# DanielaCourel/smoothed_particle_hydrodynamics

Hardware: AMD Instinct MI355X
Metric: Mparticle-steps/sec (whole node), dam-break (higher is better)
Workload: dtype f32

## Files before the change

smoothed_particle_hydrodynamics_amd/csrc/cell_build.h:

```cpp
#pragma once

#include "sph_device.h"

#define SCAN_THREADS 256
#ifndef RANK_UNROLL
#define RANK_UNROLL 4
#endif
#ifndef RANK_BIG
#define RANK_BIG 512
#endif
#define RANK_CHUNK 4096
#define RANK_BIG_BLOCKS 64
#define SCAN_ITEMS 16
#define SCAN_TILE (SCAN_THREADS * SCAN_ITEMS)

__device__ __forceinline__ void count_cell_runs(uint32_t c, bool live, int i,
                                                uint32_t* __restrict__ cell_count,
                                                uint32_t* __restrict__ slot, uint32_t trash)
{
   live = live && c != trash;
   const int lane = threadIdx.x & (SPH_WAVE - 1);
   const uint32_t prev = __shfl_up(c, 1);
   const bool head = (lane == 0) || (prev != c);
   const unsigned long long heads = __ballot(head);
   const unsigned long long below = heads & ((lane == 63) ? ~0ull : ((1ull << (lane + 1)) - 1ull));
   const int head_lane = 63 - __clzll(below);
   const unsigned long long above = (head_lane == 63) ? 0ull : (heads >> (head_lane + 1));
   const int run_len = above ? (__ffsll((long long)above)) : (SPH_WAVE - head_lane);
   uint32_t base = 0;
   if (live && head) base = atomicAdd(&cell_count[c], (uint32_t)run_len);
   base = __shfl(base, head_lane);
   if (live) slot[i] = base + (uint32_t)(lane - head_lane);
}

template <bool WRITE_VOX, bool CHECK_DEAD>
__global__ void __launch_bounds__(256)
k_hash_count(const float4* __restrict__ posm, const float4* __restrict__ velp,
             int32_t* __restrict__ meta, CellGrid g, SlabZone zone, uint32_t* __restrict__ key,
             uint32_t* __restrict__ slot, uint32_t* __restrict__ cell_count,
             int32_t* __restrict__ vox)
{
   const int i = blockIdx.x * blockDim.x + threadIdx.x;
   const bool live = i < meta[META_N_IN];
   uint32_t c = 0xffffffffu;
   if (live) {
      const float4 p = posm[i];
      int cx, cy, cz;
      c = cell_of(g, p.x, p.y, p.z, cx, cy, cz);
      const bool carried = zone.drop_ghosts && i < meta[META_N_LIVE];
      const int ob = meta[META_OWN_BEGIN], oe = meta[META_OWN_END];
      const bool was_owned = i >= ob && i < oe;
      if (CHECK_DEAD && __float_as_uint(velp[i].w) == SPH_DEAD_ID) {
         c = (uint32_t)g.ncells;
      } else if (carried && !was_owned) {
         c = (uint32_t)g.ncells;
// ... 4 lines not shown
         const int hi_begin = max(meta[META_BND_HI_BEGIN], lo_end);
         if (i >= lo_end && i < hi_begin) {
            const int plane = cell_coord(p.z, g.inv, g.nz_global);
            if ((zone.have_left && plane < zone.lo + zone.halo) ||
                (zone.have_right && plane >= zone.hi - zone.halo))
               atomicOr(&meta[META_ERRORS], 8);
         }
      }
      key[i] = c;
      if (WRITE_VOX) {
         vox[3 * i + 0] = cx;
         vox[3 * i + 1] = cy;
         vox[3 * i + 2] = cz;
      }
   }
   count_cell_runs(c, live, i, cell_count, slot, (uint32_t)g.ncells);
}

__device__ __forceinline__ uint32_t wave_inclusive_scan(uint32_t v, int lane)
{
#pragma unroll
   for (int d = 1; d < SPH_WAVE; d <<= 1) {
      uint32_t t = __shfl_up(v, d);
      if (lane >= d) v += t;
   }
   return v;
}

__device__ __forceinline__ uint32_t block_exclusive_scan(uint32_t v, uint32_t* total)
{
   __shared__ uint32_t wave_sums[SCAN_THREADS / SPH_WAVE];
// ... 3 lines not shown
   if (lane == SPH_WAVE - 1) wave_sums[w] = inc;
   __syncthreads();
   uint32_t carry = 0, tot = 0;
#pragma unroll
   for (int k = 0; k < SCAN_THREADS / SPH_WAVE; k++) {
      const uint32_t s = wave_sums[k];
      if (k < w) carry += s;
      tot += s;
   }
   __syncthreads();
   *total = tot;
   return carry + inc - v;
}

__global__ void __launch_bounds__(SCAN_THREADS)
k_scan_reduce(const uint32_t* __restrict__ count, int ncells, uint32_t* __restrict__ part)
{
   const int base = blockIdx.x * SCAN_TILE + threadIdx.x * SCAN_ITEMS;
   uint32_t s = 0;
   if (base + SCAN_ITEMS <= ncells) {
      const uint4* p = reinterpret_cast<const uint4*>(count + base);
#pragma unroll
      for (int k = 0; k < SCAN_ITEMS / 4; k++) {
         const uint4 v = p[k];
         s += v.x + v.y + v.z + v.w;
      }
   } else {
      for (int k = 0; k < SCAN_ITEMS; k++)
         if (base + k < ncells) s += count[base + k];
   }
   uint32_t total;
   block_exclusive_scan(s, &total);
   if (threadIdx.x == 0) part[blockIdx.x] = total;
}

__global__ void __launch_bounds__(SCAN_THREADS)
k_scan_final(uint32_t* __restrict__ count, int ncells, const uint32_t* __restrict__ part,
             uint32_t* __restrict__ cell_start, uint32_t* __restrict__ big_cells, uint32_t limit,
             int32_t* __restrict__ meta)
{
   if (blockIdx.x == 0 && threadIdx.x == 0) big_cells[0] = 0u;
   const int base = blockIdx.x * SCAN_TILE + threadIdx.x * SCAN_ITEMS;
   uint32_t v[SCAN_ITEMS];
   uint32_t s = 0;
   const bool empty_tile = part[blockIdx.x] == 0u;
   if (empty_tile) {
#pragma unroll
      for (int k = 0; k < SCAN_ITEMS; k++) v[k] = 0u;
   } else if (base + SCAN_ITEMS <= ncells) {
      const uint4* p = reinterpret_cast<const uint4*>(count + base);
#pragma unroll
      for (int k = 0; k < SCAN_ITEMS / 4; k++) {
         const uint4 q = p[k];
         v[4 * k + 0] = q.x;
         v[4 * k + 1] = q.y;
         v[4 * k + 2] = q.z;
         v[4 * k + 3] = q.w;
      }
   } else {
#pragma unroll
      for (int k = 0; k < SCAN_ITEMS; k++) v[k] = (base + k < ncells) ? count[base + k] : 0u;
   }
#pragma unroll
   for (int k = 0; k < SCAN_ITEMS; k++) s += v[k];
   uint32_t before = 0;
   for (int t = threadIdx.x; t < (int)blockIdx.x; t += SCAN_THREADS) before += part[t];
   uint32_t carry;
   block_exclusive_scan(before, &carry);
   uint32_t total;
   uint32_t run = carry + block_exclusive_scan(s, &total);
   if (base + SCAN_ITEMS <= ncells) {
      uint4* o = reinterpret_cast<uint4*>(cell_start + base);
      uint4* z = reinterpret_cast<uint4*>(count + base);
#pragma unroll
      for (int k = 0; k < SCAN_ITEMS / 4; k++) {
         uint4 q;
         q.x = min(run, limit); run += v[4 * k + 0];
         q.y = min(run, limit); run += v[4 * k + 1];
         q.z = min(run, limit); run += v[4 * k + 2];
         q.w = min(run, limit); run += v[4 * k + 3];
         o[k] = q;
         if ((v[4 * k + 0] | v[4 * k + 1] | v[4 * k + 2] | v[4 * k + 3]) != 0u) z[k] = make_uint4(0, 0, 0, 0);
      }
   } else {
      for (int k = 0; k < SCAN_ITEMS; k++) {
         if (base + k < ncells) {
            cell_start[base + k] = min(run, limit);
            if (v[k] != 0u) count[base + k] = 0;
            run += v[k];
         }
      }
   }
   if (base <= ncells - 1 && ncells - 1 < base + SCAN_ITEMS) {
      cell_start[ncells] = min(run, limit);
      if (run > limit) atomicOr(&meta[META_ERRORS], 4);
   }
}

__global__ void __launch_bounds__(256)
k_scatter(const uint32_t* __restrict__ key, const uint32_t* __restrict__ slot,
          const uint32_t* __restrict__ cell_start, int32_t* __restrict__ meta,
          uint32_t* __restrict__ perm, int cells_per_plane, int ncells, int own_lo, int own_hi,
          int sum_lo, int sum_hi, int bnd_lo, int bnd_hi, int32_t* __restrict__ tile_stats,
          int32_t* __restrict__ clear_a, int32_t* __restrict__ clear_b,
          uint32_t* __restrict__ big_cells, uint32_t limit)
{
   const int i = blockIdx.x * blockDim.x + threadIdx.x;
   if (tile_stats && i < TSTAT_COUNT && i != TSTAT_BLOCKS) tile_stats[i] = 0;
// ... 236 lines not shown
```

smoothed_particle_hydrodynamics_amd/csrc/common_kernels.h:

```cpp
#pragma once

#include "body_policy.h"
#include "cell_build.h"
#include "load_policy.h"
#include "obstacle_policy.h"
#include "pair_math.h"

#define RED_THREADS 256

__device__ __forceinline__ void apply_boundary(const PairConsts& k, const float pos[3], float dt,
                                               float np[3], float dist, int axis, float sgn,
                                               float nv[3])
{
   float normal[3] = {0.0f, 0.0f, 0.0f};
   normal[axis] = sgn;
   float inter[3], refl[3];
#pragma unroll
   for (int c = 0; c < 3; c++) inter[c] = pos[c] + (nv[c] * dist);
   const float dot = nv[0] * normal[0] + nv[1] * normal[1] + nv[2] * normal[2];
#pragma unroll
   for (int c = 0; c < 3; c++) refl[c] = nv[c] - ((normal[c] * dot) * 2.0f);
   const float remaining = dt - dist;
#pragma unroll
   for (int c = 0; c < 3; c++) {
// ... 183 lines not shown
   }
};

template <bool UNIT_SCALE>
__device__ __forceinline__ void integrate_particle(const PairConsts& k, float4& x, float4& v,
                                                   const float4 a, double& ke, double& pe)
{
   integrate_particle_hooked<UNIT_SCALE>(k, x, v, a, ke, pe, NoHook());
}

template <bool UNIT_SCALE, bool HASH, class Hook>
__device__ __forceinline__ void integrate_block(float4* __restrict__ posm, float4* __restrict__ velp,
                                                const float4* __restrict__ acc, const PairConsts& k,
                                                double* __restrict__ epart, const CellGrid& g,
                                                uint32_t* __restrict__ key, uint32_t* __restrict__ slot,
                                                uint32_t* __restrict__ cell_count, int p, bool live,
                                                const Hook& hook)
{
   double ke = 0.0, pe = 0.0;
   uint32_t c = 0xffffffffu;
   if (live || Hook::records) {
      float4 x = make_float4(0.0f, 0.0f, 0.0f, 0.0f), v = x, a = x;
      if (live) {
         x = posm[p];
         v = velp[p];
         a = acc[p];
      }
      integrate_particle_hooked<UNIT_SCALE>(k, x, v, a, ke, pe, hook);
      if (live) {
         posm[p] = x;
         velp[p] = v;
         if (HASH) {
            int cx, cy, cz;
            c = cell_of(g, x.x, x.y, x.z, cx, cy, cz);
            key[p] = c;
         }
      } else {
         ke = 0.0;
         pe = 0.0;
      }
   }
   if (HASH) count_cell_runs(c, live, p, cell_count, slot, (uint32_t)g.ncells);
   __shared__ double s_ke[RED_THREADS / SPH_WAVE], s_pe[RED_THREADS / SPH_WAVE];
#pragma unroll
   for (int d = SPH_WAVE / 2; d > 0; d >>= 1) {
      ke += __shfl_down(ke, d);
      pe += __shfl_down(pe, d);
   }
   const int lane = threadIdx.x & (SPH_WAVE - 1), w = threadIdx.x / SPH_WAVE;
   if (lane == 0) {
      s_ke[w] = ke;
      s_pe[w] = pe;
   }
   __syncthreads();
   if (threadIdx.x == 0) {
      double a = 0.0, b = 0.0;
#pragma unroll
      for (int q = 0; q < RED_THREADS / SPH_WAVE; q++) {
         a += s_ke[q];
         b += s_pe[q];
      }
      epart[2 * blockIdx.x + 0] = a;
      epart[2 * blockIdx.x + 1] = b;
   }
}

template <bool UNIT_SCALE, bool HASH>
__global__ void __launch_bounds__(RED_THREADS)
k_integrate(float4* __restrict__ posm, float4* __restrict__ velp, const float4* __restrict__ acc,
            const int32_t* __restrict__ meta, PairConsts k, double* __restrict__ epart, CellGrid g,
            uint32_t* __restrict__ key, uint32_t* __restrict__ slot,
            uint32_t* __restrict__ cell_count)
{
   const int p = meta[META_OWN_BEGIN] + blockIdx.x * blockDim.x + threadIdx.x;
   integrate_block<UNIT_SCALE, HASH>(posm, velp, acc, k, epart, g, key, slot, cell_count, p, p < meta[META_OWN_END], NoHook());
}

template <bool UNIT_SCALE, bool HASH>
__global__ void __launch_bounds__(RED_THREADS)
k_integrate_obst(float4* __restrict__ posm, float4* __restrict__ velp, const float4* __restrict__ acc,
                 const int32_t* __restrict__ meta, PairConsts k, double* __restrict__ epart, CellGrid g,
                 uint32_t* __restrict__ key, uint32_t* __restrict__ slot,
                 uint32_t* __restrict__ cell_count, const sph_hip_obstacle* __restrict__ obst, int n_obst)
{
   const int p = meta[META_OWN_BEGIN] + blockIdx.x * blockDim.x + threadIdx.x;
   const ObstacleHook hook = {obst, n_obst, k.dt, k.damping};
   integrate_block<UNIT_SCALE, HASH>(posm, velp, acc, k, epart, g, key, slot, cell_count, p, p < meta[META_OWN_END], hook);
}

template <bool UNIT_SCALE, bool HASH>
__global__ void __launch_bounds__(RED_THREADS)
k_integrate_loads(float4* __restrict__ posm, float4* __restrict__ velp, const float4* __restrict__ acc,
                  const int32_t* __restrict__ meta, PairConsts k, double* __restrict__ epart, CellGrid g,
                  uint32_t* __restrict__ key, uint32_t* __restrict__ slot,
                  uint32_t* __restrict__ cell_count, const sph_hip_obstacle* __restrict__ obst, int n_obst,
                  unsigned long long* __restrict__ row, int quantum_log2)
{
   const int p = meta[META_OWN_BEGIN] + blockIdx.x * blockDim.x + threadIdx.x;
   const bool live = p < meta[META_OWN_END];
   const LoadHook hook = {obst, n_obst, k.dt, k.damping, row, load_scale(quantum_log2), live};
   integrate_block<UNIT_SCALE, HASH>(posm, velp, acc, k, epart, g, key, slot, cell_count, p, live, hook);
}

template <bool UNIT_SCALE, bool HASH>
__global__ void __launch_bounds__(RED_THREADS)
k_integrate_obst_moving(float4* __restrict__ posm, float4* __restrict__ velp, const float4* __restrict__ acc,
                        const int32_t* __restrict__ meta, PairConsts k, double* __restrict__ epart, CellGrid g,
                        uint32_t* __restrict__ key, uint32_t* __restrict__ slot,
                        uint32_t* __restrict__ cell_count, const sph_hip_obstacle* __restrict__ obst, int n_obst,
                        const sph_hip_obstacle_motion* __restrict__ motion, float tau0, float tau1)
{
   const int p = meta[META_OWN_BEGIN] + blockIdx.x * blockDim.x + threadIdx.x;
   const MovingObstacleHook hook = {{obst, n_obst, k.dt, k.damping}, motion, tau0, tau1};
   integrate_block<UNIT_SCALE, HASH>(posm, velp, acc, k, epart, g, key, slot, cell_count, p, p < meta[META_OWN_END], hook);
}

template <bool UNIT_SCALE, bool HASH>
__global__ void __launch_bounds__(RED_THREADS)
k_integrate_loads_moving(float4* __restrict__ posm, float4* __restrict__ velp, const float4* __restrict__ acc,
                         const int32_t* __restrict__ meta, PairConsts k, double* __restrict__ epart, CellGrid g,
                         uint32_t* __restrict__ key, uint32_t* __restrict__ slot,
                         uint32_t* __restrict__ cell_count, const sph_hip_obstacle* __restrict__ obst, int n_obst,
                         unsigned long long* __restrict__ row, int quantum_log2,
                         const sph_hip_obstacle_motion* __restrict__ motion, float tau0, float tau1)
{
   const int p = meta[META_OWN_BEGIN] + blockIdx.x * blockDim.x + threadIdx.x;
   const bool live = p < meta[META_OWN_END];
   const MovingLoadHook hook = {{obst, n_obst, k.dt, k.damping, row, load_scale(quantum_log2), live}, motion, tau0, tau1};
   integrate_block<UNIT_SCALE, HASH>(posm, velp, acc, k, epart, g, key, slot, cell_count, p, live, hook);
}

__global__ void __launch_bounds__(SPH_WAVE)
k_bodies_advance(const sph_hip_body* __restrict__ bodies, BodyState* __restrict__ state, int n_obst,
                 const unsigned long long* row, int quantum_log2, float dt, unsigned long long* clear)
{
   const int lane = threadIdx.x;
   if (clear)
      for (int w = lane; w < LOAD_ROW_WORDS; w += SPH_WAVE) clear[w] = 0ull;
   if (lane >= n_obst) return;
   const sph_hip_body b = bodies[lane];
   BodyState s = state[lane];
   body_advance(b, s, reinterpret_cast<const long long*>(row), lane, quantum_log2, dt);
   state[lane] = s;
}

template <bool UNIT_SCALE, bool HASH>
__global__ void __launch_bounds__(RED_THREADS)
k_integrate_bodies(float4* __restrict__ posm, float4* __restrict__ velp, const float4* __restrict__ acc,
                   const int32_t* __restrict__ meta, PairConsts k, double* __restrict__ epart, CellGrid g,
                   uint32_t* __restrict__ key, uint32_t* __restrict__ slot,
                   uint32_t* __restrict__ cell_count, const sph_hip_obstacle* __restrict__ obst, int n_obst,
                   unsigned long long* __restrict__ row, int quantum_log2,
                   const sph_hip_obstacle_motion* __restrict__ motion, float tau0, float tau1,
                   const sph_hip_body* __restrict__ bodies, const BodyState* __restrict__ state)
{
   const int p = meta[META_OWN_BEGIN] + blockIdx.x * blockDim.x + threadIdx.x;
   const bool live = p < meta[META_OWN_END];
   const BodyLoadHook hook = {{obst, n_obst, k.dt, k.damping, row, load_scale(quantum_log2), live}, motion, tau0, tau1,
                              bodies, state};
   integrate_block<UNIT_SCALE, HASH>(posm, velp, acc, k, epart, g, key, slot, cell_count, p, live, hook);
}

__global__ void __launch_bounds__(RED_THREADS)
k_energy_total(const double* __restrict__ epart, int nblocks, double* __restrict__ out)
{
   double ke = 0.0, pe = 0.0;
   for (int b = threadIdx.x; b < nblocks; b += RED_THREADS) {
      ke += epart[2 * b + 0];
      pe += epart[2 * b + 1];
   }
   __shared__ double s_ke[RED_THREADS], s_pe[RED_THREADS];
   s_ke[threadIdx.x] = ke;
   s_pe[threadIdx.x] = pe;
   __syncthreads();
   for (int d = RED_THREADS / 2; d > 0; d >>= 1) {
// ... 106 lines not shown
```

smoothed_particle_hydrodynamics_amd/csrc/context.h:

```cpp
#pragma once

#include <stdlib.h>
#include <string.h>

#include <memory>
#include <new>
#include <utility>

#include "cell_build.h"
#include "common_kernels.h"
#include "full_kernels.h"
#include "full_tiled.h"
#include "ref_kernels.h"
#include "sample_kernels.h"
#include "surface_kernels.h"
#include "render_kernels.h"
#include "slab_kernels.h"
#include "slab_rccl.h"

namespace {

std::string g_create_error;

inline int div_up(int a, int b) { return (a + b - 1) / b; }
// ... 117 lines not shown
   long long ev_steps = 0;
   std::string err;

   CellGrid grid;

   DevBuf<float4> posm[2];
   DevBuf<float4> velp[2];
   int cur = 0;

   DevBuf<uint32_t> key;
   DevBuf<uint32_t> slot;
   DevBuf<uint32_t> perm;
   DevBuf<uint32_t> order;
   DevBuf<uint32_t> cell_count;
   DevBuf<uint32_t> cell_start;
   DevBuf<uint32_t> scan_part;
   DevBuf<uint32_t> big_cells;
   int scan_tiles = 0;

   DevBuf<float> rho;
   DevBuf<float4> velB;
   DevBuf<float> auxc;
   DevBuf<float4> acc;
   DevBuf<int32_t> ncount;
   DevBuf<TileDesc> tile_desc;
   DevBuf<uint32_t> nlist;
   DevBuf<uint32_t> nlist_overflow;
   int fast = 0;
   struct {
      int valid = 0;
      int fast = 0;
      float rho0 = 0.0f, stiffness = 0.0f, kernel3 = 0.0f;
   } terms;
// ... 119 lines not shown
   if (count <= cap) return SPH_HIP_OK;
   SPH_TRY(hipStreamSynchronize(ctx->stream));
   buf.reset();
   cap = 0;
   if (!capacity_err) {
      SPH_TRY(dev_alloc(buf, count));
   } else if (dev_alloc(buf, count) != hipSuccess) {
      (void)hipGetLastError();
      ctx->err = capacity_err;
      return SPH_HIP_ERR_CAPACITY;
   }
   cap = count;
   return SPH_HIP_OK;
}

bool loads_pending(const sph_hip_context* ctx) { return ctx->loads_next < ctx->loads_rows; }

int check_ctx(sph_hip_context* ctx)
{
   if (!ctx) return SPH_HIP_ERR_INVALID;
   hipError_t e = hipSetDevice(ctx->device);
   if (e != hipSuccess) {
      ctx->err = std::string("hipSetDevice: ") + hipGetErrorString(e);
      return SPH_HIP_ERR_DEVICE;
   }
   return SPH_HIP_OK;
}

int create_impl(sph_hip_context** out, const sph_hip_params* params, int capacity, int mode,
                int device, int plane_lo, int plane_hi, int halo)
// ... 82 lines not shown
   CREATE_TRY(hipSetDevice(device));
   CREATE_TRY(hipStreamCreateWithFlags(ctx->own_stream.out(), hipStreamNonBlocking));
   ctx->stream = ctx->own_stream;
   for (auto& slot : ctx->ev)
      for (Event& ev : slot) CREATE_TRY(hipEventCreate(ev.out()));
   for (int k = 0; k < 2; k++) CREATE_TRY(event_create(ctx->ev_pace[k]));
   const size_t cap = (size_t)capacity;
   const int nbuf = (mode == SPH_HIP_MODE_FULL) ? 2 : 1;
   for (int b = 0; b < nbuf; b++) {
      CREATE_TRY(dev_alloc(ctx->posm[b], cap));
      CREATE_TRY(dev_alloc(ctx->velp[b], cap));
   }
   CREATE_TRY(dev_alloc(ctx->key, cap));
   CREATE_TRY(dev_alloc(ctx->slot, cap));
   CREATE_TRY(dev_alloc(ctx->perm, cap));
   const size_t cells_padded = (size_t)ctx->scan_tiles * SCAN_TILE + 16;
   CREATE_TRY(dev_alloc(ctx->cell_count, cells_padded));
   CREATE_TRY(dev_alloc(ctx->cell_start, cells_padded));
   CREATE_TRY(dev_alloc(ctx->scan_part, (size_t)ctx->scan_tiles + 1));
   CREATE_TRY(dev_alloc(ctx->big_cells, cap / RANK_BIG + 2));
   CREATE_TRY(hipMemsetAsync(ctx->big_cells, 0, sizeof(uint32_t), ctx->stream));
   CREATE_TRY(hipMemsetAsync(ctx->cell_count, 0, cells_padded * sizeof(uint32_t), ctx->stream));
   CREATE_TRY(hipMemsetAsync(ctx->cell_start, 0, cells_padded * sizeof(uint32_t), ctx->stream));
   CREATE_TRY(dev_alloc(ctx->rho, cap));
   CREATE_TRY(dev_alloc(ctx->acc, cap));
   CREATE_TRY(dev_alloc(ctx->ncount, cap));
   CREATE_TRY(hipMemsetAsync(ctx->rho, 0, cap * sizeof(float), ctx->stream));
   CREATE_TRY(hipMemsetAsync(ctx->acc, 0, cap * sizeof(float4), ctx->stream));
   CREATE_TRY(hipMemsetAsync(ctx->ncount, 0, cap * sizeof(int32_t), ctx->stream));
   CREATE_TRY(dev_alloc(ctx->meta, META_COUNT));
   CREATE_TRY(hipMemsetAsync(ctx->meta, 0, META_COUNT * sizeof(int32_t), ctx->stream));
   if (mode == SPH_HIP_MODE_FULL) {
      CREATE_TRY(dev_alloc(ctx->velB, cap));
      CREATE_TRY(dev_alloc(ctx->auxc, cap));
      CREATE_TRY(dev_alloc(ctx->tile_desc, (size_t)div_up(capacity, TILE_THREADS) + 1));
      ctx->list_cap = NLIST_CAP;
      ctx->list_cap_max = NLIST_CAP_MAX;
      if (const char* v = getenv("SPH_HIP_LIST_CAP")) {
// ... 67 lines not shown
```

smoothed_particle_hydrodynamics_amd/csrc/full_tiled.h:

```cpp
#pragma once

#include "launch_policy.h"
#include "common_kernels.h"
#include "full_kernels.h"
#include "neighbor_lists.h"
#include "slab_kernels.h"

#if defined(SPH_ABLATE) && !defined(SPH_DIAGNOSTIC_BUILD)
#error "SPH_ABLATE is for diagnostic builds only: add -DSPH_DIAGNOSTIC_BUILD (tools/build_variant.sh does)"
#endif

#ifdef SPH_TRIPCOUNT
#ifndef SPH_DIAGNOSTIC_BUILD
#error "SPH_TRIPCOUNT is for diagnostic builds only: add -DSPH_DIAGNOSTIC_BUILD"
#endif
enum {
   TRIP_D_WAVES = 0, TRIP_D_CHUNKS_W, TRIP_D_TEST8_W, TRIP_D_TEST8_L, TRIP_D_SLOTS_L, TRIP_D_POPS_W,
   TRIP_D_POPS_L, TRIP_D_POPLOOPS_W, TRIP_D_SUMTRIPS_W, TRIP_D_SUMSLOTS_W, TRIP_D_LISTED_L, TRIP_D_LANES_L,
   TRIP_A_WAVES = 16, TRIP_A_PTRIPS_W, TRIP_A_CNT_L, TRIP_A_VTRIPS_W, TRIP_A_NV_L, TRIP_A_LANES_L,
   TRIP_COUNT = 32
};
__device__ unsigned long long g_trip[TRIP_COUNT];
struct TripCounters {
   unsigned int v[16];
// ... 708 lines not shown
                                                const CellGrid& g, int p, bool live, float4 x,
                                                float4 a, int wg_index)
{
   double ke = 0.0, pe = 0.0;
   uint32_t c = 0xffffffffu;
   float4 v = make_float4(0.f, 0.f, 0.f, 0.f);
   if (live) {
      v = fs.velp_in[p];
      integrate_particle<UNIT_SCALE>(k, x, v, a, ke, pe);
      fs.posm_out[p] = x;
      fs.velp_out[p] = v;
      int cx, cy, cz;
      c = cell_of(g, x.x, x.y, x.z, cx, cy, cz);
      fs.key[p] = c;
   }
   count_cell_runs(c, live, p, fs.cell_count, fs.slot, (uint32_t)g.ncells);
   if (fs.slab) {
      bool to_left = false, to_right = false;
      if (live) {
         const int ob = fs.meta[META_OWN_BEGIN], oe = fs.meta[META_OWN_END];
         const int lo_end = min(fs.meta[META_BND_LO_END], oe);
         const int hi_begin = min(max(fs.meta[META_BND_HI_BEGIN], lo_end), oe);
         const int plane = cell_coord(x.z, g.inv, g.nz_global);
         const bool near_left = fs.zone.have_left && plane < fs.zone.lo + fs.zone.halo;
         const bool near_right = fs.zone.have_right && plane >= fs.zone.hi - fs.zone.halo;
         if ((p >= ob && p < lo_end) || (p >= hi_begin && p < oe)) {
            to_left = near_left;
            to_right = near_right;
         } else if (near_left || near_right) {
            atomicOr(&fs.meta[META_ERRORS], 8);
         }
// ... 445 lines not shown
```

smoothed_particle_hydrodynamics_amd/csrc/launch.h:

```cpp
#pragma once

#include <math.h>

#include <type_traits>

#include "context.h"

namespace {

template <class F>
void bind_flags(F&& f) { f(); }
template <class F, class... Rest>
void bind_flags(F&& f, bool flag, Rest... rest)
{
   if (flag) bind_flags([&](auto... later) { f(std::true_type{}, later...); }, rest...);
   else bind_flags([&](auto... later) { f(std::false_type{}, later...); }, rest...);
}

PairConsts pair_consts(const sph_hip_params& p, bool fast)
{
   PairConsts k;
   k.h2 = p.h2;
   static const float screen = getenv("SPH_HIP_TEST_SCREEN") ? (float)atof(getenv("SPH_HIP_TEST_SCREEN"))
                                                             : TEST_SCREEN_FACTOR;
// ... 161 lines not shown
}

int launch_cell_build(sph_hip_context* ctx, void* clear_left = nullptr, void* clear_right = nullptr,
                      bool keep_sums = false)
{
   const int n = ctx->n;
   if (n == 0) return SPH_HIP_OK;
   const int blocks = div_up(n, 256);
   const CellGrid g = ctx->grid;
   hipStream_t st = ctx->stream;
   const int cur = ctx->cur;
   const SlabZone zone = slab_zone(ctx);
   if (ctx->prehashed == 2) {
      ctx->prehashed = 0;
      hipLaunchKernelGGL(k_hash_tail, dim3(SLAB_PACK_BLOCKS), dim3(256), 0, st, ctx->posm[cur], ctx->meta, g,
                         ctx->key, ctx->slot, ctx->cell_count);
   } else if (ctx->prehashed) {
      ctx->prehashed = 0;
   } else {
      const bool ref = ctx->mode == SPH_HIP_MODE_REF;
      bind_flags([&](auto R, auto D) {
         if constexpr (!(R.value && D.value))
            hipLaunchKernelGGL((k_hash_count<R.value, D.value>), dim3(blocks), dim3(256), 0, st, ctx->posm[cur],
                               ctx->velp[cur], ctx->meta, g, zone, ctx->key, ctx->slot, ctx->cell_count,
                               R.value ? ctx->vox.get() : nullptr);
      }, ref, !ref && ctx->may_hold_dead != 0);
   }
   ctx->early_exchange = 0;
   ctx->may_hold_dead = 0;
   const int tiles = ctx->scan_tiles;
   const int ncells_scan = g.ncells + 1;
   hipLaunchKernelGGL(k_scan_reduce, dim3(tiles), dim3(SCAN_THREADS), 0, st, ctx->cell_count,
                      ncells_scan, ctx->scan_part);
   hipLaunchKernelGGL(k_scan_final, dim3(tiles), dim3(SCAN_THREADS), 0, st, ctx->cell_count,
                      ncells_scan, ctx->scan_part, ctx->cell_start, ctx->big_cells, (uint32_t)ctx->capacity,
                      ctx->meta);
   const PlaneRanges r = plane_ranges(ctx->plane_lo, ctx->plane_hi, g.z0, g.nz, ctx->halo, zone.have_left,
                                      zone.have_right);
   hipLaunchKernelGGL(k_scatter, dim3(blocks), dim3(256), 0, st, ctx->key, ctx->slot,
                      ctx->cell_start, ctx->meta, ctx->perm, g.nx * g.ny, g.ncells, r.own_lo, r.own_hi,
                      r.sum_lo, r.sum_hi, r.bnd_lo, r.bnd_hi, ctx->tile_stats, (int32_t*)clear_left,
                      (int32_t*)clear_right, ctx->big_cells, (uint32_t)ctx->capacity);
   uint32_t* scratch_key = reinterpret_cast<uint32_t*>(ctx->stage.get());
   uint32_t* scratch_src = scratch_key + ctx->capacity;
   uint32_t* remap = (keep_sums && ctx->mode == SPH_HIP_MODE_FULL && !ctx->had_exchange) ? ctx->slot : nullptr;
   if (ctx->mode == SPH_HIP_MODE_REF) {
      hipLaunchKernelGGL(k_rank_order, dim3(blocks), dim3(256), 0, st, ctx->perm, ctx->key,
                         ctx->cell_start, ctx->meta, ctx->order);
      hipLaunchKernelGGL(k_rank_big<false>, dim3(RANK_BIG_BLOCKS), dim3(256), 0, st, ctx->big_cells,
                         ctx->perm, ctx->cell_start, (const float4*)nullptr, (const float4*)nullptr,
                         (float4*)nullptr, (float4*)nullptr, ctx->order, scratch_key, scratch_src,
// ... 98 lines not shown

void launch_accel_lists(sph_hip_context* ctx, bool unit, int blocks, const PairConsts& k, int part,
                        hipStream_t st, bool fused = false, const SlabFused* slab = nullptr)
{
   FusedStep fs;
   memset(&fs, 0, sizeof(fs));
   if (fused) {
      fs.on = 1;
      fs.velp_in = ctx->velp[ctx->cur];
      fs.posm_out = ctx->posm[ctx->cur ^ 1];
      fs.velp_out = ctx->velp[ctx->cur ^ 1];
      fs.epart = ctx->epart + 2;
      fs.key = ctx->key;
      fs.slot = ctx->slot;
      fs.cell_count = ctx->cell_count;
      if (slab) {
         fs.slab = 1;
         fs.zone = slab_zone(ctx);
         fs.left = (SlabMsg*)slab->left;
         fs.right = (SlabMsg*)slab->right;
         fs.msg_capacity = slab->capacity;
         fs.meta = ctx->meta;
      }
   }
   const int cap = ctx->caps.cap_accel;
   const size_t lds = (size_t)(cap + TILE_PAD) * ACCEL_TILE_BYTES;
   bind_flags([&](auto U, auto M, auto W, auto F) {
      if constexpr (M.value || !F.value)
      hipLaunchKernelGGL((k_full_accel_lists<U.value, M.value, W.value, F.value>), dim3(blocks),
                         dim3(TILE_THREADS), lds, st, ctx->posm[ctx->cur], ctx->velB, ctx->rho, ctx->auxc,
// ... 117 lines not shown
         ctx->body_flip ^= 1;
         load_row = clear = ctx->body_rows.get() + (size_t)ctx->body_flip * LOAD_ROW_WORDS;
      }
      hipLaunchKernelGGL(k_bodies_advance, dim3(1), dim3(SPH_WAVE), 0, ctx->stream, ctx->bodies_dev, ctx->body_state_dev,
                         ctx->n_obst, ctx->body_last_row, ctx->body_quantum, ctx->prm.time_step, clear);
      ctx->body_last_row = load_row;
      if (n == 0) SPH_TRY(hipGetLastError());
   }
   if (n == 0) return SPH_HIP_OK;
   const PairConsts k = pair_consts(ctx->prm, ctx->fast != 0);
   const int blocks = div_up(n, RED_THREADS);
   bind_flags([&](auto U, auto H) {
      if (bodies)
         hipLaunchKernelGGL((k_integrate_bodies<U.value, H.value>), dim3(blocks), dim3(RED_THREADS), 0, ctx->stream,
                            ctx->posm[ctx->cur], ctx->velp[ctx->cur], ctx->acc, ctx->meta, k, ctx->epart + 2,
                            ctx->grid, ctx->key, ctx->slot, ctx->cell_count, ctx->obst_dev, ctx->n_obst,
                            load_row, ctx->body_quantum, ctx->n_motion > 0 ? ctx->motion_dev.get() : nullptr, tau0, tau1,
                            ctx->bodies_dev, ctx->body_state_dev);
      else if (moving && load_row)
         hipLaunchKernelGGL((k_integrate_loads_moving<U.value, H.value>), dim3(blocks), dim3(RED_THREADS), 0, ctx->stream,
                            ctx->posm[ctx->cur], ctx->velp[ctx->cur], ctx->acc, ctx->meta, k, ctx->epart + 2,
                            ctx->grid, ctx->key, ctx->slot, ctx->cell_count, ctx->obst_dev, ctx->n_obst,
                            load_row, ctx->loads_quantum, ctx->motion_dev, tau0, tau1);
      else if (moving)
         hipLaunchKernelGGL((k_integrate_obst_moving<U.value, H.value>), dim3(blocks), dim3(RED_THREADS), 0, ctx->stream,
                            ctx->posm[ctx->cur], ctx->velp[ctx->cur], ctx->acc, ctx->meta, k, ctx->epart + 2,
                            ctx->grid, ctx->key, ctx->slot, ctx->cell_count, ctx->obst_dev, ctx->n_obst,
                            ctx->motion_dev, tau0, tau1);
      else if (load_row)
         hipLaunchKernelGGL((k_integrate_loads<U.value, H.value>), dim3(blocks), dim3(RED_THREADS), 0, ctx->stream,
                            ctx->posm[ctx->cur], ctx->velp[ctx->cur], ctx->acc, ctx->meta, k, ctx->epart + 2,
                            ctx->grid, ctx->key, ctx->slot, ctx->cell_count, ctx->obst_dev, ctx->n_obst,
                            load_row, ctx->loads_quantum);
      else if (ctx->n_obst > 0)
         hipLaunchKernelGGL((k_integrate_obst<U.value, H.value>), dim3(blocks), dim3(RED_THREADS), 0, ctx->stream,
                            ctx->posm[ctx->cur], ctx->velp[ctx->cur], ctx->acc, ctx->meta, k, ctx->epart + 2,
                            ctx->grid, ctx->key, ctx->slot, ctx->cell_count, ctx->obst_dev, ctx->n_obst);
      else
         hipLaunchKernelGGL((k_integrate<U.value, H.value>), dim3(blocks), dim3(RED_THREADS), 0, ctx->stream,
                            ctx->posm[ctx->cur], ctx->velp[ctx->cur], ctx->acc, ctx->meta, k, ctx->epart + 2,
                            ctx->grid, ctx->key, ctx->slot, ctx->cell_count);
   }, unit_scale(ctx->prm), with_hash);
   ctx->energy_blocks = blocks;
   ctx->prehashed = with_hash ? 1 : 0;
   SPH_TRY(hipGetLastError());
   return SPH_HIP_OK;
}

void fused_step_done(sph_hip_context* ctx, int prehashed)
{
   ctx->cur ^= 1;
   ctx->energy_blocks = div_up(ctx->n, TILE_THREADS);
   ctx->prehashed = prehashed;
}

int drop_prehash(sph_hip_context* ctx)
{
   if (!ctx->prehashed) return SPH_HIP_OK;
   ctx->prehashed = 0;
   SPH_TRY(hipMemsetAsync(ctx->cell_count, 0, ((size_t)ctx->scan_tiles * SCAN_TILE + 16) * sizeof(uint32_t),
                          ctx->stream));
   return SPH_HIP_OK;
}

int pace_host(sph_hip_context* ctx)
{
   const long long k = ctx->steps_enqueued++;
   if (k % PACE_STEPS != 0) return SPH_HIP_OK;
   const int slot = (int)((k / PACE_STEPS) & 1);
   if (k >= 2 * PACE_STEPS) SPH_TRY(hipEventSynchronize(ctx->ev_pace[slot]));
   SPH_TRY(hipEventRecord(ctx->ev_pace[slot], ctx->stream));
   return SPH_HIP_OK;
}

struct StepEvents {
   Event* ev;
// ... 88 lines not shown
```

smoothed_particle_hydrodynamics_amd/csrc/slab_kernels.h:

```cpp
#pragma once

#include "common_kernels.h"
#include "sph_device.h"

#define SLAB_HEADER_INTS 8
#define SLAB_PACK_BLOCKS 4096

struct SlabMsg {
   int32_t header[SLAB_HEADER_INTS];
   float4 rec[1];
};

__device__ __forceinline__ int msg_reserve(int32_t* __restrict__ counter, bool want)
{
   const unsigned long long m = __ballot(want);
   if (m == 0ull) return -1;
   const int lane = threadIdx.x & (SPH_WAVE - 1);
   const int leader = __ffsll((long long)m) - 1;
   int base = 0;
   if (lane == leader) base = atomicAdd(counter, __popcll(m));
   base = __shfl(base, leader);
   return want ? base + __popcll(m & ((1ull << lane) - 1ull)) : -1;
}

// ... 99 lines not shown
template <bool UNIT_SCALE>
__global__ void __launch_bounds__(256)
k_slab_pack_early_obst_moving(const float4* __restrict__ posm, const float4* __restrict__ velp,
                              const float4* __restrict__ acc, int32_t* __restrict__ meta, PairConsts k,
                              CellGrid g, SlabZone zone, SlabMsg* __restrict__ left,
                              SlabMsg* __restrict__ right, int capacity,
                              const sph_hip_obstacle* __restrict__ obst, int n_obst,
                              const sph_hip_obstacle_motion* __restrict__ motion, float tau0, float tau1)
{
   const MovingObstacleHook hook = {{obst, n_obst, k.dt, k.damping}, motion, tau0, tau1};
   slab_pack_early<UNIT_SCALE>(posm, velp, acc, meta, k, g, zone, left, right, capacity, hook);
}

__global__ void __launch_bounds__(256)
k_hash_tail(const float4* __restrict__ posm, int32_t* __restrict__ meta, CellGrid g,
            uint32_t* __restrict__ key, uint32_t* __restrict__ slot, uint32_t* __restrict__ cell_count)
{
   const int ob = meta[META_OWN_BEGIN], oe = meta[META_OWN_END];
   const int n_live = meta[META_N_LIVE], n_in = meta[META_N_IN];
   const int todo = ob + (n_in - oe);
   for (int q0 = blockIdx.x * blockDim.x; q0 < todo; q0 += gridDim.x * blockDim.x) {
      const int q = q0 + threadIdx.x;
      const bool live = q < todo;
      const int i = q < ob ? q : oe + (q - ob);
      uint32_t c = 0xffffffffu;
      if (live) {
         if (i < n_live) {
            c = (uint32_t)g.ncells;
         } else {
            const float4 p = posm[i];
            int cx, cy, cz;
            c = cell_of(g, p.x, p.y, p.z, cx, cy, cz);
            if (c == (uint32_t)g.ncells) atomicOr(&meta[META_ERRORS], 1);
         }
         key[i] = c;
      }
      count_cell_runs(c, live, i, cell_count, slot, (uint32_t)g.ncells);
   }
}

__global__ void __launch_bounds__(256)
k_export_records(const float4* __restrict__ posm, const float4* __restrict__ velp,
                 const int32_t* __restrict__ meta, float4* __restrict__ rec)
{
   const int ob = meta[META_OWN_BEGIN];
   const int p = ob + blockIdx.x * blockDim.x + threadIdx.x;
   if (p >= meta[META_OWN_END]) return;
   rec[2 * (p - ob)] = posm[p];
   rec[2 * (p - ob) + 1] = velp[p];
}

__global__ void __launch_bounds__(256)
// ... 31 lines not shown
```

smoothed_particle_hydrodynamics_amd/csrc/sph_device.h:

```cpp
#pragma once

#include <hip/hip_runtime.h>
#include <stdint.h>

#include <string>

#include "../../include/sph_hip.h"
#include "launch_policy.h"

#define SPH_WAVE 64
#define EV_RING 128
#define PACE_STEPS 16

#define SPH_TRY(expr)                                                                \
   do {                                                                              \
      hipError_t e_ = (expr);                                                        \
      if (e_ != hipSuccess) {                                                        \
         ctx->err = std::string(#expr) + ": " + hipGetErrorString(e_);               \
         return SPH_HIP_ERR_DEVICE;                                                  \
      }                                                                              \
   } while (0)

struct CellGrid {
   int nx, ny, nz;
// ... 23 lines not shown
   int drop_ghosts;
   int early;
};

#define TEST_SCREEN_FACTOR 1.000002f
struct SlabMsg;
struct FusedStep {
   int on;
   const float4* velp_in;
   float4* posm_out;
   float4* velp_out;
   double* epart;
   uint32_t* key;
   uint32_t* slot;
   uint32_t* cell_count;
   int slab;
   SlabZone zone;
   SlabMsg* left;
   SlabMsg* right;
   int msg_capacity;
   int32_t* meta;
};
#define SPH_DEAD_ID 0xffffffffu

struct PairConsts {
   float h2, hscaled, hscaled2, sim_scale;
   float h2_screen;
   float fast_k2s, fast_unscale;
   float kernel1, kernel2, kernel3;
   float rho0, stiffness, viscosity;
// ... 91 lines not shown
```

Before: 4723.

## Accumulate per-tile totals during hashing and drop scan reduce pass

Hashing kernels now also accumulate per-scan-tile particle totals through wave-aggregated atomics into a double-buffered array stored after cell_count. This removes the separate k_scan_reduce kernel, which read the whole cell_count array each step. k_scan_final uses these totals directly, zeroes the other buffer for the next step, and takes a fast path for empty tiles that only writes cell_start. The cost is extra ballot loops and atomics in every hash site.

Measured after the change: 4720. Within noise of the previous version (-0.1%).

```diff
diff --git a/smoothed_particle_hydrodynamics_amd/csrc/cell_build.h b/smoothed_particle_hydrodynamics_amd/csrc/cell_build.h
--- a/smoothed_particle_hydrodynamics_amd/csrc/cell_build.h
+++ b/smoothed_particle_hydrodynamics_amd/csrc/cell_build.h
@@ -16,6 +16,7 @@
 
 __device__ __forceinline__ void count_cell_runs(uint32_t c, bool live, int i,
                                                 uint32_t* __restrict__ cell_count,
+                                                uint32_t* __restrict__ tile_total,
                                                 uint32_t* __restrict__ slot, uint32_t trash)
 {
    live = live && c != trash;
@@ -31,6 +32,15 @@
    if (live && head) base = atomicAdd(&cell_count[c], (uint32_t)run_len);
    base = __shfl(base, head_lane);
    if (live) slot[i] = base + (uint32_t)(lane - head_lane);
+   const uint32_t tile = live ? c / SCAN_TILE : 0xffffffffu;
+   unsigned long long todo = __ballot(live);
+   while (todo) {
+      const int first = __ffsll((long long)todo) - 1;
+      const uint32_t t = __builtin_amdgcn_readlane(tile, first);
+      const unsigned long long same = __ballot(tile == t);
+      if (lane == first) atomicAdd(&tile_total[t], (uint32_t)__popcll(same));
+      todo &= ~same;
+   }
 }
 
 template <bool WRITE_VOX, bool CHECK_DEAD>
@@ -38,7 +48,7 @@
 k_hash_count(const float4* __restrict__ posm, const float4* __restrict__ velp,
              int32_t* __restrict__ meta, CellGrid g, SlabZone zone, uint32_t* __restrict__ key,
              uint32_t* __restrict__ slot, uint32_t* __restrict__ cell_count,
-             int32_t* __restrict__ vox)
+             uint32_t* __restrict__ tile_total, int32_t* __restrict__ vox)
 {
    const int i = blockIdx.x * blockDim.x + threadIdx.x;
    const bool live = i < meta[META_N_IN];
@@ -73,7 +83,7 @@
          vox[3 * i + 2] = cz;
       }
    }
-   count_cell_runs(c, live, i, cell_count, slot, (uint32_t)g.ncells);
+   count_cell_runs(c, live, i, cell_count, tile_total, slot, (uint32_t)g.ncells);
 }
 
 __device__ __forceinline__ uint32_t wave_inclusive_scan(uint32_t v, int lane)
@@ -107,40 +117,22 @@
 }
 
 __global__ void __launch_bounds__(SCAN_THREADS)
-k_scan_reduce(const uint32_t* __restrict__ count, int ncells, uint32_t* __restrict__ part)
-{
+k_scan_final(uint32_t* __restrict__ count, int ncells, const uint32_t* __restrict__ total,
+             uint32_t* __restrict__ total_next, uint32_t* __restrict__ cell_start,
+             uint32_t* __restrict__ big_cells, uint32_t limit, int32_t* __restrict__ meta)
+{
+   if (blockIdx.x == 0 && threadIdx.x == 0) big_cells[0] = 0u;
+   if (threadIdx.x == 0) total_next[blockIdx.x] = 0u;
    const int base = blockIdx.x * SCAN_TILE + threadIdx.x * SCAN_ITEMS;
-   uint32_t s = 0;
-   if (base + SCAN_ITEMS <= ncells) {
-      const uint4* p = reinterpret_cast<const uint4*>(count + base);
-#pragma unroll
-      for (int k = 0; k < SCAN_ITEMS / 4; k++) {
-         const uint4 v = p[k];
-         s += v.x + v.y + v.z + v.w;
-      }
-   } else {
-      for (int k = 0; k < SCAN_ITEMS; k++)
-         if (base + k < ncells) s += count[base + k];
-   }
-   uint32_t total;
-   block_exclusive_scan(s, &total);
-   if (threadIdx.x == 0) part[blockIdx.x] = total;
-}
-
-__global__ void __launch_bounds__(SCAN_THREADS)
-k_scan_final(uint32_t* __restrict__ count, int ncells, const uint32_t* __restrict__ part,
-             uint32_t* __restrict__ cell_start, uint32_t* __restrict__ big_cells, uint32_t limit,
-             int32_t* __restrict__ meta)
-{
-   if (blockIdx.x == 0 && threadIdx.x == 0) big_cells[0] = 0u;
-   const int base = blockIdx.x * SCAN_TILE + threadIdx.x * SCAN_ITEMS;
+   const bool whole = base + SCAN_ITEMS <= ncells;
+   const bool last = base <= ncells - 1 && ncells - 1 < base + SCAN_ITEMS;
+   const bool empty_tile = total[blockIdx.x] == 0u;
    uint32_t v[SCAN_ITEMS];
    uint32_t s = 0;
-   const bool empty_tile = part[blockIdx.x] == 0u;
    if (empty_tile) {
 #pragma unroll
       for (int k = 0; k < SCAN_ITEMS; k++) v[k] = 0u;
-   } else if (base + SCAN_ITEMS <= ncells) {
+   } else if (whole) {
       const uint4* p = reinterpret_cast<const uint4*>(count + base);
 #pragma unroll
       for (int k = 0; k < SCAN_ITEMS / 4; k++) {
@@ -154,15 +146,31 @@
 #pragma unroll
       for (int k = 0; k < SCAN_ITEMS; k++) v[k] = (base + k < ncells) ? count[base + k] : 0u;
    }
-#pragma unroll
-   for (int k = 0; k < SCAN_ITEMS; k++) s += v[k];
    uint32_t before = 0;
-   for (int t = threadIdx.x; t < (int)blockIdx.x; t += SCAN_THREADS) before += part[t];
+   for (int t = threadIdx.x; t < (int)blockIdx.x; t += SCAN_THREADS) before += total[t];
    uint32_t carry;
    block_exclusive_scan(before, &carry);
-   uint32_t total;
-   uint32_t run = carry + block_exclusive_scan(s, &total);
-   if (base + SCAN_ITEMS <= ncells) {
+   if (empty_tile) {
+      const uint32_t first = min(carry, limit);
+      if (whole) {
+         uint4* o = reinterpret_cast<uint4*>(cell_start + base);
+#pragma unroll
+         for (int k = 0; k < SCAN_ITEMS / 4; k++) o[k] = make_uint4(first, first, first, first);
+      } else {
+         for (int k = 0; k < SCAN_ITEMS; k++)
+            if (base + k < ncells) cell_start[base + k] = first;
+      }
+      if (last) {
+         cell_start[ncells] = first;
+         if (carry > limit) atomicOr(&meta[META_ERRORS], 4);
+      }
+      return;
+   }
+#pragma unroll
+   for (int k = 0; k < SCAN_ITEMS; k++) s += v[k];
+   uint32_t sum;
+   uint32_t run = carry + block_exclusive_scan(s, &sum);
+   if (whole) {
       uint4* o = reinterpret_cast<uint4*>(cell_start + base);
       uint4* z = reinterpret_cast<uint4*>(count + base);
 #pragma unroll
@@ -184,7 +192,7 @@
          }
       }
    }
-   if (base <= ncells - 1 && ncells - 1 < base + SCAN_ITEMS) {
+   if (last) {
       cell_start[ncells] = min(run, limit);
       if (run > limit) atomicOr(&meta[META_ERRORS], 4);
    }
diff --git a/smoothed_particle_hydrodynamics_amd/csrc/common_kernels.h b/smoothed_particle_hydrodynamics_amd/csrc/common_kernels.h
--- a/smoothed_particle_hydrodynamics_amd/csrc/common_kernels.h
+++ b/smoothed_particle_hydrodynamics_amd/csrc/common_kernels.h
@@ -221,7 +221,8 @@
                                                 const float4* __restrict__ acc, const PairConsts& k,
                                                 double* __restrict__ epart, const CellGrid& g,
                                                 uint32_t* __restrict__ key, uint32_t* __restrict__ slot,
-                                                uint32_t* __restrict__ cell_count, int p, bool live,
+                                                uint32_t* __restrict__ cell_count,
+                                                uint32_t* __restrict__ tile_total, int p, bool live,
                                                 const Hook& hook)
 {
    double ke = 0.0, pe = 0.0;
@@ -247,7 +248,7 @@
          pe = 0.0;
       }
    }
-   if (HASH) count_cell_runs(c, live, p, cell_count, slot, (uint32_t)g.ncells);
+   if (HASH) count_cell_runs(c, live, p, cell_count, tile_total, slot, (uint32_t)g.ncells);
    __shared__ double s_ke[RED_THREADS / SPH_WAVE], s_pe[RED_THREADS / SPH_WAVE];
 #pragma unroll
    for (int d = SPH_WAVE / 2; d > 0; d >>= 1) {
@@ -277,10 +278,10 @@
 k_integrate(float4* __restrict__ posm, float4* __restrict__ velp, const float4* __restrict__ acc,
             const int32_t* __restrict__ meta, PairConsts k, double* __restrict__ epart, CellGrid g,
             uint32_t* __restrict__ key, uint32_t* __restrict__ slot,
-            uint32_t* __restrict__ cell_count)
-{
-   const int p = meta[META_OWN_BEGIN] + blockIdx.x * blockDim.x + threadIdx.x;
-   integrate_block<UNIT_SCALE, HASH>(posm, velp, acc, k, epart, g, key, slot, cell_count, p, p < meta[META_OWN_END], NoHook());
+            uint32_t* __restrict__ cell_count, uint32_t* __restrict__ tile_total)
+{
+   const int p = meta[META_OWN_BEGIN] + blockIdx.x * blockDim.x + threadIdx.x;
+   integrate_block<UNIT_SCALE, HASH>(posm, velp, acc, k, epart, g, key, slot, cell_count, tile_total, p, p < meta[META_OWN_END], NoHook());
 }
 
 template <bool UNIT_SCALE, bool HASH>
@@ -288,11 +289,12 @@
 k_integrate_obst(float4* __restrict__ posm, float4* __restrict__ velp, const float4* __restrict__ acc,
                  const int32_t* __restrict__ meta, PairConsts k, double* __restrict__ epart, CellGrid g,
                  uint32_t* __restrict__ key, uint32_t* __restrict__ slot,
-                 uint32_t* __restrict__ cell_count, const sph_hip_obstacle* __restrict__ obst, int n_obst)
+                 uint32_t* __restrict__ cell_count, uint32_t* __restrict__ tile_total,
+                 const sph_hip_obstacle* __restrict__ obst, int n_obst)
 {
    const int p = meta[META_OWN_BEGIN] + blockIdx.x * blockDim.x + threadIdx.x;
    const ObstacleHook hook = {obst, n_obst, k.dt, k.damping};
-   integrate_block<UNIT_SCALE, HASH>(posm, velp, acc, k, epart, g, key, slot, cell_count, p, p < meta[META_OWN_END], hook);
+   integrate_block<UNIT_SCALE, HASH>(posm, velp, acc, k, epart, g, key, slot, cell_count, tile_total, p, p < meta[META_OWN_END], hook);
 }
 
 template <bool UNIT_SCALE, bool HASH>
@@ -300,13 +302,14 @@
 k_integrate_loads(float4* __restrict__ posm, float4* __restrict__ velp, const float4* __restrict__ acc,
                   const int32_t* __restrict__ meta, PairConsts k, double* __restrict__ epart, CellGrid g,
                   uint32_t* __restrict__ key, uint32_t* __restrict__ slot,
-                  uint32_t* __restrict__ cell_count, const sph_hip_obstacle* __restrict__ obst, int n_obst,
+                  uint32_t* __restrict__ cell_count, uint32_t* __restrict__ tile_total,
+                  const sph_hip_obstacle* __restrict__ obst, int n_obst,
                   unsigned long long* __restrict__ row, int quantum_log2)
 {
    const int p = meta[META_OWN_BEGIN] + blockIdx.x * blockDim.x + threadIdx.x;
    const bool live = p < meta[META_OWN_END];
    const LoadHook hook = {obst, n_obst, k.dt, k.damping, row, load_scale(quantum_log2), live};
-   integrate_block<UNIT_SCALE, HASH>(posm, velp, acc, k, epart, g, key, slot, cell_count, p, live, hook);
+   integrate_block<UNIT_SCALE, HASH>(posm, velp, acc, k, epart, g, key, slot, cell_count, tile_total, p, live, hook);
 }
 
 template <bool UNIT_SCALE, bool HASH>
@@ -314,12 +317,13 @@
 k_integrate_obst_moving(float4* __restrict__ posm, float4* __restrict__ velp, const float4* __restrict__ acc,
                         const int32_t* __restrict__ meta, PairConsts k, double* __restrict__ epart, CellGrid g,
                         uint32_t* __restrict__ key, uint32_t* __restrict__ slot,
-                        uint32_t* __restrict__ cell_count, const sph_hip_obstacle* __restrict__ obst, int n_obst,
+                        uint32_t* __restrict__ cell_count, uint32_t* __restrict__ tile_total,
+                        const sph_hip_obstacle* __restrict__ obst, int n_obst,
                         const sph_hip_obstacle_motion* __restrict__ motion, float tau0, float tau1)
 {
    const int p = meta[META_OWN_BEGIN] + blockIdx.x * blockDim.x + threadIdx.x;
    const MovingObstacleHook hook = {{obst, n_obst, k.dt, k.damping}, motion, tau0, tau1};
-   integrate_block<UNIT_SCALE, HASH>(posm, velp, acc, k, epart, g, key, slot, cell_count, p, p < meta[META_OWN_END], hook);
+   integrate_block<UNIT_SCALE, HASH>(posm, velp, acc, k, epart, g, key, slot, cell_count, tile_total, p, p < meta[META_OWN_END], hook);
 }
 
 template <bool UNIT_SCALE, bool HASH>
@@ -327,14 +331,15 @@
 k_integrate_loads_moving(float4* __restrict__ posm, float4* __restrict__ velp, const float4* __restrict__ acc,
                          const int32_t* __restrict__ meta, PairConsts k, double* __restrict__ epart, CellGrid g,
                          uint32_t* __restrict__ key, uint32_t* __restrict__ slot,
-                         uint32_t* __restrict__ cell_count, const sph_hip_obstacle* __restrict__ obst, int n_obst,
+                         uint32_t* __restrict__ cell_count, uint32_t* __restrict__ tile_total,
+                         const sph_hip_obstacle* __restrict__ obst, int n_obst,
                          unsigned long long* __restrict__ row, int quantum_log2,
                          const sph_hip_obstacle_motion* __restrict__ motion, float tau0, float tau1)
 {
    const int p = meta[META_OWN_BEGIN] + blockIdx.x * blockDim.x + threadIdx.x;
    const bool live = p < meta[META_OWN_END];
    const MovingLoadHook hook = {{obst, n_obst, k.dt, k.damping, row, load_scale(quantum_log2), live}, motion, tau0, tau1};
-   integrate_block<UNIT_SCALE, HASH>(posm, velp, acc, k, epart, g, key, slot, cell_count, p, live, hook);
+   integrate_block<UNIT_SCALE, HASH>(posm, velp, acc, k, epart, g, key, slot, cell_count, tile_total, p, live, hook);
 }
 
 __global__ void __launch_bounds__(SPH_WAVE)
@@ -356,7 +361,8 @@
 k_integrate_bodies(float4* __restrict__ posm, float4* __restrict__ velp, const float4* __restrict__ acc,
                    const int32_t* __restrict__ meta, PairConsts k, double* __restrict__ epart, CellGrid g,
                    uint32_t* __restrict__ key, uint32_t* __restrict__ slot,
-                   uint32_t* __restrict__ cell_count, const sph_hip_obstacle* __restrict__ obst, int n_obst,
+                   uint32_t* __restrict__ cell_count, uint32_t* __restrict__ tile_total,
+                   const sph_hip_obstacle* __restrict__ obst, int n_obst,
                    unsigned long long* __restrict__ row, int quantum_log2,
                    const sph_hip_obstacle_motion* __restrict__ motion, float tau0, float tau1,
                    const sph_hip_body* __restrict__ bodies, const BodyState* __restrict__ state)
@@ -365,7 +371,7 @@
    const bool live = p < meta[META_OWN_END];
    const BodyLoadHook hook = {{obst, n_obst, k.dt, k.damping, row, load_scale(quantum_log2), live}, motion, tau0, tau1,
                               bodies, state};
-   integrate_block<UNIT_SCALE, HASH>(posm, velp, acc, k, epart, g, key, slot, cell_count, p, live, hook);
+   integrate_block<UNIT_SCALE, HASH>(posm, velp, acc, k, epart, g, key, slot, cell_count, tile_total, p, live, hook);
 }
 
 __global__ void __launch_bounds__(RED_THREADS)
diff --git a/smoothed_particle_hydrodynamics_amd/csrc/context.h b/smoothed_particle_hydrodynamics_amd/csrc/context.h
--- a/smoothed_particle_hydrodynamics_amd/csrc/context.h
+++ b/smoothed_particle_hydrodynamics_amd/csrc/context.h
@@ -155,9 +155,9 @@
    DevBuf<uint32_t> order;
    DevBuf<uint32_t> cell_count;
    DevBuf<uint32_t> cell_start;
-   DevBuf<uint32_t> scan_part;
    DevBuf<uint32_t> big_cells;
    int scan_tiles = 0;
+   int totals_cur = 0;
 
    DevBuf<float> rho;
    DevBuf<float4> velB;
@@ -307,6 +307,13 @@
    return SPH_HIP_OK;
 }
 
+size_t cells_padded(const sph_hip_context* ctx) { return (size_t)ctx->scan_tiles * SCAN_TILE + 16; }
+size_t count_words(const sph_hip_context* ctx) { return cells_padded(ctx) + 2 * (size_t)ctx->scan_tiles; }
+uint32_t* tile_totals(const sph_hip_context* ctx, int which)
+{
+   return ctx->cell_count.get() + cells_padded(ctx) + (size_t)which * ctx->scan_tiles;
+}
+
 bool loads_pending(const sph_hip_context* ctx) { return ctx->loads_next < ctx->loads_rows; }
 
 int check_ctx(sph_hip_context* ctx)
@@ -419,14 +426,12 @@
    CREATE_TRY(dev_alloc(ctx->key, cap));
    CREATE_TRY(dev_alloc(ctx->slot, cap));
    CREATE_TRY(dev_alloc(ctx->perm, cap));
-   const size_t cells_padded = (size_t)ctx->scan_tiles * SCAN_TILE + 16;
-   CREATE_TRY(dev_alloc(ctx->cell_count, cells_padded));
-   CREATE_TRY(dev_alloc(ctx->cell_start, cells_padded));
-   CREATE_TRY(dev_alloc(ctx->scan_part, (size_t)ctx->scan_tiles + 1));
+   CREATE_TRY(dev_alloc(ctx->cell_count, count_words(ctx.get())));
+   CREATE_TRY(dev_alloc(ctx->cell_start, cells_padded(ctx.get())));
    CREATE_TRY(dev_alloc(ctx->big_cells, cap / RANK_BIG + 2));
    CREATE_TRY(hipMemsetAsync(ctx->big_cells, 0, sizeof(uint32_t), ctx->stream));
-   CREATE_TRY(hipMemsetAsync(ctx->cell_count, 0, cells_padded * sizeof(uint32_t), ctx->stream));
-   CREATE_TRY(hipMemsetAsync(ctx->cell_start, 0, cells_padded * sizeof(uint32_t), ctx->stream));
+   CREATE_TRY(hipMemsetAsync(ctx->cell_count, 0, count_words(ctx.get()) * sizeof(uint32_t), ctx->stream));
+   CREATE_TRY(hipMemsetAsync(ctx->cell_start, 0, cells_padded(ctx.get()) * sizeof(uint32_t), ctx->stream));
    CREATE_TRY(dev_alloc(ctx->rho, cap));
    CREATE_TRY(dev_alloc(ctx->acc, cap));
    CREATE_TRY(dev_alloc(ctx->ncount, cap));
diff --git a/smoothed_particle_hydrodynamics_amd/csrc/full_tiled.h b/smoothed_particle_hydrodynamics_amd/csrc/full_tiled.h
--- a/smoothed_particle_hydrodynamics_amd/csrc/full_tiled.h
+++ b/smoothed_particle_hydrodynamics_amd/csrc/full_tiled.h
@@ -746,7 +746,7 @@
       c = cell_of(g, x.x, x.y, x.z, cx, cy, cz);
       fs.key[p] = c;
    }
-   count_cell_runs(c, live, p, fs.cell_count, fs.slot, (uint32_t)g.ncells);
+   count_cell_runs(c, live, p, fs.cell_count, fs.tile_total, fs.slot, (uint32_t)g.ncells);
    if (fs.slab) {
       bool to_left = false, to_right = false;
       if (live) {
diff --git a/smoothed_particle_hydrodynamics_amd/csrc/launch.h b/smoothed_particle_hydrodynamics_amd/csrc/launch.h
--- a/smoothed_particle_hydrodynamics_amd/csrc/launch.h
+++ b/smoothed_particle_hydrodynamics_amd/csrc/launch.h
@@ -199,7 +199,7 @@
    if (ctx->prehashed == 2) {
       ctx->prehashed = 0;
       hipLaunchKernelGGL(k_hash_tail, dim3(SLAB_PACK_BLOCKS), dim3(256), 0, st, ctx->posm[cur], ctx->meta, g,
-                         ctx->key, ctx->slot, ctx->cell_count);
+                         ctx->key, ctx->slot, ctx->cell_count, tile_totals(ctx, ctx->totals_cur));
    } else if (ctx->prehashed) {
       ctx->prehashed = 0;
    } else {
@@ -208,18 +208,17 @@
          if constexpr (!(R.value && D.value))
             hipLaunchKernelGGL((k_hash_count<R.value, D.value>), dim3(blocks), dim3(256), 0, st, ctx->posm[cur],
                                ctx->velp[cur], ctx->meta, g, zone, ctx->key, ctx->slot, ctx->cell_count,
-                               R.value ? ctx->vox.get() : nullptr);
+                               tile_totals(ctx, ctx->totals_cur), R.value ? ctx->vox.get() : nullptr);
       }, ref, !ref && ctx->may_hold_dead != 0);
    }
    ctx->early_exchange = 0;
    ctx->may_hold_dead = 0;
    const int tiles = ctx->scan_tiles;
    const int ncells_scan = g.ncells + 1;
-   hipLaunchKernelGGL(k_scan_reduce, dim3(tiles), dim3(SCAN_THREADS), 0, st, ctx->cell_count,
-                      ncells_scan, ctx->scan_part);
    hipLaunchKernelGGL(k_scan_final, dim3(tiles), dim3(SCAN_THREADS), 0, st, ctx->cell_count,
-                      ncells_scan, ctx->scan_part, ctx->cell_start, ctx->big_cells, (uint32_t)ctx->capacity,
-                      ctx->meta);
+                      ncells_scan, tile_totals(ctx, ctx->totals_cur), tile_totals(ctx, ctx->totals_cur ^ 1),
+                      ctx->cell_start, ctx->big_cells, (uint32_t)ctx->capacity, ctx->meta);
+   ctx->totals_cur ^= 1;
    const PlaneRanges r = plane_ranges(ctx->plane_lo, ctx->plane_hi, g.z0, g.nz, ctx->halo, zone.have_left,
                                       zone.have_right);
    hipLaunchKernelGGL(k_scatter, dim3(blocks), dim3(256), 0, st, ctx->key, ctx->slot,
@@ -348,6 +347,7 @@
       fs.key = ctx->key;
       fs.slot = ctx->slot;
       fs.cell_count = ctx->cell_count;
+      fs.tile_total = tile_totals(ctx, ctx->totals_cur);
       if (slab) {
          fs.slab = 1;
          fs.zone = slab_zone(ctx);
@@ -495,32 +495,32 @@
       if (bodies)
          hipLaunchKernelGGL((k_integrate_bodies<U.value, H.value>), dim3(blocks), dim3(RED_THREADS), 0, ctx->stream,
                             ctx->posm[ctx->cur], ctx->velp[ctx->cur], ctx->acc, ctx->meta, k, ctx->epart + 2,
-                            ctx->grid, ctx->key, ctx->slot, ctx->cell_count, ctx->obst_dev, ctx->n_obst,
+                            ctx->grid, ctx->key, ctx->slot, ctx->cell_count, tile_totals(ctx, ctx->totals_cur), ctx->obst_dev, ctx->n_obst,
                             load_row, ctx->body_quantum, ctx->n_motion > 0 ? ctx->motion_dev.get() : nullptr, tau0, tau1,
                             ctx->bodies_dev, ctx->body_state_dev);
       else if (moving && load_row)
          hipLaunchKernelGGL((k_integrate_loads_moving<U.value, H.value>), dim3(blocks), dim3(RED_THREADS), 0, ctx->stream,
                             ctx->posm[ctx->cur], ctx->velp[ctx->cur], ctx->acc, ctx->meta, k, ctx->epart + 2,
-                            ctx->grid, ctx->key, ctx->slot, ctx->cell_count, ctx->obst_dev, ctx->n_obst,
+                            ctx->grid, ctx->key, ctx->slot, ctx->cell_count, tile_totals(ctx, ctx->totals_cur), ctx->obst_dev, ctx->n_obst,
                             load_row, ctx->loads_quantum, ctx->motion_dev, tau0, tau1);
       else if (moving)
          hipLaunchKernelGGL((k_integrate_obst_moving<U.value, H.value>), dim3(blocks), dim3(RED_THREADS), 0, ctx->stream,
                             ctx->posm[ctx->cur], ctx->velp[ctx->cur], ctx->acc, ctx->meta, k, ctx->epart + 2,
-                            ctx->grid, ctx->key, ctx->slot, ctx->cell_count, ctx->obst_dev, ctx->n_obst,
+                            ctx->grid, ctx->key, ctx->slot, ctx->cell_count, tile_totals(ctx, ctx->totals_cur), ctx->obst_dev, ctx->n_obst,
                             ctx->motion_dev, tau0, tau1);
       else if (load_row)
          hipLaunchKernelGGL((k_integrate_loads<U.value, H.value>), dim3(blocks), dim3(RED_THREADS), 0, ctx->stream,
                             ctx->posm[ctx->cur], ctx->velp[ctx->cur], ctx->acc, ctx->meta, k, ctx->epart + 2,
-                            ctx->grid, ctx->key, ctx->slot, ctx->cell_count, ctx->obst_dev, ctx->n_obst,
+                            ctx->grid, ctx->key, ctx->slot, ctx->cell_count, tile_totals(ctx, ctx->totals_cur), ctx->obst_dev, ctx->n_obst,
                             load_row, ctx->loads_quantum);
       else if (ctx->n_obst > 0)
          hipLaunchKernelGGL((k_integrate_obst<U.value, H.value>), dim3(blocks), dim3(RED_THREADS), 0, ctx->stream,
                             ctx->posm[ctx->cur], ctx->velp[ctx->cur], ctx->acc, ctx->meta, k, ctx->epart + 2,
-                            ctx->grid, ctx->key, ctx->slot, ctx->cell_count, ctx->obst_dev, ctx->n_obst);
+                            ctx->grid, ctx->key, ctx->slot, ctx->cell_count, tile_totals(ctx, ctx->totals_cur), ctx->obst_dev, ctx->n_obst);
       else
          hipLaunchKernelGGL((k_integrate<U.value, H.value>), dim3(blocks), dim3(RED_THREADS), 0, ctx->stream,
                             ctx->posm[ctx->cur], ctx->velp[ctx->cur], ctx->acc, ctx->meta, k, ctx->epart + 2,
-                            ctx->grid, ctx->key, ctx->slot, ctx->cell_count);
+                            ctx->grid, ctx->key, ctx->slot, ctx->cell_count, tile_totals(ctx, ctx->totals_cur));
    }, unit_scale(ctx->prm), with_hash);
    ctx->energy_blocks = blocks;
    ctx->prehashed = with_hash ? 1 : 0;
@@ -539,8 +539,7 @@
 {
    if (!ctx->prehashed) return SPH_HIP_OK;
    ctx->prehashed = 0;
-   SPH_TRY(hipMemsetAsync(ctx->cell_count, 0, ((size_t)ctx->scan_tiles * SCAN_TILE + 16) * sizeof(uint32_t),
-                          ctx->stream));
+   SPH_TRY(hipMemsetAsync(ctx->cell_count, 0, count_words(ctx) * sizeof(uint32_t), ctx->stream));
    return SPH_HIP_OK;
 }
 
diff --git a/smoothed_particle_hydrodynamics_amd/csrc/slab_kernels.h b/smoothed_particle_hydrodynamics_amd/csrc/slab_kernels.h
--- a/smoothed_particle_hydrodynamics_amd/csrc/slab_kernels.h
+++ b/smoothed_particle_hydrodynamics_amd/csrc/slab_kernels.h
@@ -137,7 +137,8 @@
 
 __global__ void __launch_bounds__(256)
 k_hash_tail(const float4* __restrict__ posm, int32_t* __restrict__ meta, CellGrid g,
-            uint32_t* __restrict__ key, uint32_t* __restrict__ slot, uint32_t* __restrict__ cell_count)
+            uint32_t* __restrict__ key, uint32_t* __restrict__ slot, uint32_t* __restrict__ cell_count,
+            uint32_t* __restrict__ tile_total)
 {
    const int ob = meta[META_OWN_BEGIN], oe = meta[META_OWN_END];
    const int n_live = meta[META_N_LIVE], n_in = meta[META_N_IN];
@@ -158,7 +159,7 @@
          }
          key[i] = c;
       }
-      count_cell_runs(c, live, i, cell_count, slot, (uint32_t)g.ncells);
+      count_cell_runs(c, live, i, cell_count, tile_total, slot, (uint32_t)g.ncells);
    }
 }
 
diff --git a/smoothed_particle_hydrodynamics_amd/csrc/sph_device.h b/smoothed_particle_hydrodynamics_amd/csrc/sph_device.h
--- a/smoothed_particle_hydrodynamics_amd/csrc/sph_device.h
+++ b/smoothed_particle_hydrodynamics_amd/csrc/sph_device.h
@@ -61,6 +61,7 @@
    uint32_t* key;
    uint32_t* slot;
    uint32_t* cell_count;
+   uint32_t* tile_total;
    int slab;
    SlabZone zone;
    SlabMsg* left;
```
